# chrischoy/DeepGlobalRegistration

Hardware: AMD Instinct MI355X
Metric: pair registrations/sec (FCGF x2 + 1-NN + 6-D inlier net + gate + weighted Procrustes + SE(3) refinement) (higher is better)
Workload: dtype f32 results via 2 x f16 split operands (3 f16 MFMA products per MAC, f32 accumulate); k = 1 convs, kNN re-evaluation and registration in exact f32, SVD in f64

## Files before the change

deepglobalregistration_amd/csrc/kmap.hip:

```cpp
#include <string.h>

#include <algorithm>

#include "dgr_internal.h"
#include "hash.h"

constexpr int KM_THREADS = 256;

template <int D>
__device__ __forceinline__ void offset_of(int k, int ks, int ts, int32_t *delta) {
  const int half = ks >> 1;
#pragma unroll
  for (int d = 0; d < D; ++d) {
    delta[d] = ((k % ks) - half) * ts;
    k /= ks;
  }
}

template <int D>
__device__ __forceinline__ int probe(const int32_t *__restrict__ out_coords, int64_t o,
                                     const int32_t *delta, const int32_t *__restrict__ in_coords,
                                     const int32_t *__restrict__ in_table, uint32_t in_mask) {
  constexpr int NC = D + 1;
  int32_t q[NC];
  q[0] = out_coords[o * NC];
#pragma unroll
  for (int d = 0; d < D; ++d) q[1 + d] = out_coords[o * NC + 1 + d] + delta[d];
  return dgr_lookup<NC>(in_table, in_mask, in_coords, q);
}

template <int D>
__global__ void __launch_bounds__(KM_THREADS)
    kmap_search(const int32_t *__restrict__ out_coords, const int32_t *n_out_dev,
                const int32_t *__restrict__ in_coords, const int32_t *__restrict__ in_table,
                uint32_t in_mask, int ks, int ts_in, int RB, int64_t n_cap, int32_t *__restrict__ hits,
                int32_t *__restrict__ block_counts, int KW, uint32_t *mask_out, uint32_t *mask_in) {
  __shared__ int wave_cnt[KM_THREADS / 64];
  const int rb = blockIdx.x, k = blockIdx.y;
  const int n_out = *n_out_dev;
  if (rb * KM_THREADS >= n_out) {
    if (threadIdx.x == 0) block_counts[(int64_t)k * RB + rb] = 0;
    return;
  }
  int32_t delta[D];
  offset_of<D>(k, ks, ts_in, delta);
  const int64_t o = (int64_t)rb * KM_THREADS + threadIdx.x;
  int hit = -1;
  if (o < n_out) {
    hit = probe<D>(out_coords, o, delta, in_coords, in_table, in_mask);
    hits[(int64_t)k * n_cap + o] = hit;
    if (hit >= 0) {
      atomicOr(&mask_out[o * KW + (k >> 5)], 1u << (k & 31));
      if (mask_in) atomicOr(&mask_in[(int64_t)hit * KW + (k >> 5)], 1u << (k & 31));
    }
  }
  unsigned long long m = __ballot(hit >= 0);
  if ((threadIdx.x & 63) == 0) wave_cnt[threadIdx.x >> 6] = __popcll(m);
  __syncthreads();
  if (threadIdx.x == 0) {
    int s = 0;
#pragma unroll
    for (int w = 0; w < KM_THREADS / 64; ++w) s += wave_cnt[w];
    block_counts[(int64_t)k * RB + rb] = s;
  }
}

__device__ __forceinline__ int mask_rank(const uint32_t *__restrict__ m, int k) {
  int r = 0;
  const int w = k >> 5;
  for (int i = 0; i < w; ++i) r += __popc(m[i]);
  return r + __popc(m[w] & ((1u << (k & 31)) - 1u));
}

__global__ void mask_count_kernel(const uint32_t *__restrict__ mask, int KW, const int32_t *n_dev, int64_t n_cap,
                                  int32_t *__restrict__ cnt, unsigned short *__restrict__ wpre = nullptr) {
  const int64_t r = (int64_t)blockIdx.x * blockDim.x + threadIdx.x;
  if (r >= n_cap) return;
  int c = 0;
  if (r < *n_dev)
    for (int i = 0; i < KW; ++i) {
      if (wpre) wpre[r * KW + i] = (unsigned short)c;
      c += __popc(mask[r * KW + i]);
    }
  cnt[r] = c;
}
constexpr int KM_MC_JOBS = 8;
struct MaskCountJobs {
  const uint32_t *mask[KM_MC_JOBS];
  const int32_t *n_dev[KM_MC_JOBS];
  long long n_cap[KM_MC_JOBS];
  int32_t *cnt[KM_MC_JOBS];
  unsigned short *wpre[KM_MC_JOBS];
};
template <int KW>
__global__ void mask_count_multi(MaskCountJobs J) {
  const int m = blockIdx.y;
  const int64_t r = (int64_t)blockIdx.x * blockDim.x + threadIdx.x;
  if (r >= J.n_cap[m]) return;
  int c = 0;
  if (r < *J.n_dev[m]) {
    uint32_t w[KW];
#pragma unroll
    for (int i = 0; i < KW; ++i) w[i] = J.mask[m][r * KW + i];
#pragma unroll
    for (int i = 0; i < KW; ++i) {
      J.wpre[m][r * KW + i] = (unsigned short)c;
      c += __popc(w[i]);
    }
  }
  J.cnt[m][r] = c;
}
__device__ __forceinline__ int mask_rank_pre(const uint32_t *__restrict__ m, const unsigned short *__restrict__ pre, int k) {
  return pre[k >> 5] + __popc(m[k >> 5] & ((1u << (k & 31)) - 1u));
}


__device__ __forceinline__ unsigned long long hit_pack(int k, int64_t o, int64_t in) {
  return ((unsigned long long)k << 54) | ((unsigned long long)o << 27) | (unsigned long long)in;
}
constexpr int KM_REGION = 512;
constexpr int KM_JOBS6 = 8;
struct HitList {
  unsigned long long *recs;
  int32_t *wave_count;
  int region;
};
__device__ __forceinline__ void hit_begin(volatile int *cur) {
  if ((threadIdx.x & 63) == 0) cur[threadIdx.x >> 6] = 0;
}
__device__ __forceinline__ int64_t hit_slots(int n, const HitList &h, volatile int *cur, int wave_id) {
  const unsigned long long act = __ballot(1), two = __ballot(n == 2);
  const int lane = threadIdx.x & 63, w = threadIdx.x >> 6;
  const unsigned long long below = (1ull << lane) - 1ull;
  int base = 0;
  if (lane == __ffsll((long long)act) - 1) {
    base = cur[w];
    const int need = __popcll(act) + __popcll(two);
    if (base >= 0 && base + need <= h.region) {
      cur[w] = base + need;
    } else {
      cur[w] = -1;
      base = -1;
    }
  }
  base = __builtin_amdgcn_readfirstlane(base);
  if (base < 0) return -1;
  return (int64_t)wave_id * h.region + base + __popcll(act & below) + __popcll(two & below);
}
__device__ __forceinline__ void hit_end(const HitList &h, volatile int *cur, int wave_id) {
  if ((threadIdx.x & 63) == 0) h.wave_count[wave_id] = cur[threadIdx.x >> 6];
}

struct PrunedArgs {
  const int32_t *out_coords, *n_out_dev;
  const int4 *out_order;
  int64_t n_cap;
  DgrHalfBuckets hb;
  int ts_in, symmetric;
};
template <class Emit>
__device__ __forceinline__ void pruned_search6(const PrunedArgs &a, int64_t t, Emit &&emit) {
  const int NJ = a.symmetric ? 14 : 27;
  const int ts_in = a.ts_in;
  const int ja = (int)(t / a.n_cap);
  const int64_t p = t - (int64_t)ja * a.n_cap;
  int b = -1;
  int64_t o = 0;
  int c4 = 0, c5 = 0, c6 = 0;
  if (ja < NJ && p < *a.n_out_dev) {
    const int4 me = a.out_order[p];
    o = me.w; c4 = me.x; c5 = me.y; c6 = me.z;
    const int32_t *co = a.out_coords + o * 7;
    int32_t q[4];
    q[0] = co[0];
    q[1] = co[1] + ((ja % 3) - 1) * ts_in;
    q[2] = co[2] + (((ja / 3) % 3) - 1) * ts_in;
    q[3] = co[3] + ((ja / 9) - 1) * ts_in;
    b = dgr_lookup<4>(a.hb.table, a.hb.mask, a.hb.bkeys, q);
  }
  const int beg = b >= 0 ? a.hb.start[b] : 0, end = b >= 0 ? a.hb.start[b + 1] : 0;
  for (int p0 = beg; p0 < end; p0 += 4) {
    int4 e[4];
#pragma unroll
    for (int u = 0; u < 4; ++u) e[u] = a.hb.second[min(p0 + u, end - 1)];
#pragma unroll
    for (int u = 0; u < 4; ++u) {
      if (p0 + u >= end) break;
      const int d4 = e[u].x - c4, d5 = e[u].y - c5, d6 = e[u].z - c6;
      if (abs(d4) <= ts_in && abs(d5) <= ts_in && abs(d6) <= ts_in) {
        const int k = ja + 27 * ((d4 / ts_in + 1) + 3 * (d5 / ts_in + 1) + 9 * (d6 / ts_in + 1));
        if (a.symmetric && ja == 13 && k > 364) continue;
        emit(k, o, e[u].w);
      }
    }
  }
}

struct Bits6Jobs {
  PrunedArgs pa[KM_JOBS6];
  uint32_t *mask_out[KM_JOBS6], *mask_in[KM_JOBS6];
  HitList hl[KM_JOBS6];
  int blocks[KM_JOBS6];
};
__global__ void __launch_bounds__(KM_THREADS)
    kmap_bits_pruned6(Bits6Jobs J, int KW) {
  __shared__ int hit_cur[KM_THREADS / 64];
  const int jm = blockIdx.y;
  if ((int)blockIdx.x >= J.blocks[jm]) return;
  const PrunedArgs a = J.pa[jm];
  uint32_t *const mask_out = J.mask_out[jm], *const mask_in = J.mask_in[jm];
  const HitList hl = J.hl[jm];
  hit_begin(hit_cur);
  const int wid = (int)(blockIdx.x * (KM_THREADS / 64) + (threadIdx.x >> 6));
  pruned_search6(a, (int64_t)blockIdx.x * KM_THREADS + threadIdx.x, [&](int k, int64_t o, int in) {
    atomicOr(&mask_out[o * KW + (k >> 5)], 1u << (k & 31));
    const int km = 728 - k;
    if (a.symmetric) {
      if (km != k) atomicOr(&mask_out[(int64_t)in * KW + (km >> 5)], 1u << (km & 31));
    } else if (mask_in) {
      atomicOr(&mask_in[(int64_t)in * KW + (k >> 5)], 1u << (k & 31));
    }
    const int n = (a.symmetric && km != k) ? 2 : 1;
    const int64_t s = hit_slots(n, hl, hit_cur, wid);
    if (s >= 0) {
      hl.recs[s] = hit_pack(k, o, in);
      if (n == 2) hl.recs[s + 1] = hit_pack(km, in, o);
    }
  });
  hit_end(hl, hit_cur, wid);
}

constexpr int KM_KMAX = 736;
struct Colmask6Jobs {
  const uint32_t *mask_out[KM_JOBS6];
  const int32_t *n_out_dev[KM_JOBS6];
  int RB[KM_JOBS6];
  int4 *cell[KM_JOBS6];
  int32_t *counts[KM_JOBS6], *row_cnt[KM_JOBS6];
  unsigned short *wpre[KM_JOBS6];
};
__global__ void __launch_bounds__(KM_THREADS)
    kmap_colmask(Colmask6Jobs J, int K, int KW) {
  __shared__ unsigned long long bal[KM_THREADS / 64][KM_KMAX];
  const int jm = blockIdx.y;
  const int RB = J.RB[jm];
  if ((int)blockIdx.x >= RB) return;
  const uint32_t *__restrict__ mask_out = J.mask_out[jm];
  const int32_t *n_out_dev = J.n_out_dev[jm];
  int4 *__restrict__ cell = J.cell[jm];
  int32_t *__restrict__ counts = J.counts[jm], *__restrict__ row_cnt = J.row_cnt[jm];
  unsigned short *__restrict__ wpre = J.wpre[jm];
  const int rb = blockIdx.x;
  const int lane = threadIdx.x & 63, wave = threadIdx.x >> 6;
  const int n_out = *n_out_dev;
  const int64_t o = (int64_t)rb * KM_THREADS + threadIdx.x;
  int row_pairs = 0;
  constexpr int KW_MAX = (KM_KMAX + 31) / 32;
  uint32_t words[KW_MAX];
#pragma unroll
  for (int w = 0; w < KW_MAX; ++w) words[w] = (w < KW && o < n_out) ? mask_out[o * KW + w] : 0u;
#pragma unroll
  for (int w = 0; w < KW_MAX; ++w) {
    if (w < KW) {
      const uint32_t word = words[w];
      if (o < n_out) wpre[o * KW + w] = (unsigned short)row_pairs;
      row_pairs += __popc(word);
      unsigned long long mine = 0;
#pragma unroll
      for (int b = 0; b < 32; ++b) {
        const unsigned long long m = __ballot((word >> b) & 1u);
        if (lane == b) mine = m;
      }
      if (lane < 32 && 32 * w + lane < KM_KMAX) bal[wave][32 * w + lane] = mine;
    }
  }
  if (o < n_out) row_cnt[o] = row_pairs;
  __syncthreads();
  for (int k = threadIdx.x; k < K; k += KM_THREADS) {
    int run = 0;
#pragma unroll
    for (int g = 0; g < KM_THREADS / 64; ++g) {
      const unsigned long long m = bal[g][k];
      cell[((int64_t)rb * (KM_THREADS / 64) + g) * K + k] = make_int4((int)(m & 0xffffffffull), (int)(m >> 32), run, 0);
      run += __popcll(m);
    }
    counts[(int64_t)k * RB + rb] = run;
  }
}

struct PlaceArgs {
  int K, KW, RB;
  const uint32_t *mask_out;
  const int32_t *out_ptr;
  const int4 *cell;
  const int32_t *base;
  int32_t *pair_in, *pair_out;
  uint16_t *pair_k;
  int32_t *out_pos;
  int64_t pair_cap;
  int32_t *overflow;
  const uint32_t *mask_in;
  const int32_t *in_ptr;
  int32_t *in_pos;
  const unsigned short *wpre_out, *wpre_in;
};
__device__ __forceinline__ void place_pair(const PlaceArgs &p, int k, int64_t o, int64_t in) {
  const int64_t slot = (int64_t)p.out_ptr[o] + mask_rank_pre(p.mask_out + o * p.KW, p.wpre_out + o * p.KW, k);
  const int64_t g = o >> 6;
  const int4 c = p.cell[g * p.K + k];
  const unsigned long long cm = ((unsigned long long)(uint32_t)c.y << 32) | (uint32_t)c.x;
  const int64_t pos = (int64_t)p.base[(int64_t)k * p.RB + (g >> 2)] + c.z + __popcll(cm & ((1ull << (o & 63)) - 1ull));
  if (pos < p.pair_cap && slot < p.pair_cap) {
    p.pair_in[pos] = (int32_t)in;
    if (p.pair_out) p.pair_out[pos] = (int32_t)o;
    if (p.pair_k) p.pair_k[pos] = (uint16_t)k;
    p.out_pos[slot] = (int32_t)pos;
    if (p.mask_in) p.in_pos[p.in_ptr[in] + mask_rank_pre(p.mask_in + in * p.KW, p.wpre_in + in * p.KW, k)] = (int32_t)pos;
  } else {
    *p.overflow = 2;
  }
}

struct Place6Jobs {
  HitList h[KM_JOBS6];
  PlaceArgs p[KM_JOBS6];
  PrunedArgs replay[KM_JOBS6];
  int n_waves[KM_JOBS6], blocks[KM_JOBS6];
};
__global__ void __launch_bounds__(KM_THREADS)
    kmap_place_hits(Place6Jobs J) {
  const int jm = blockIdx.y;
  const int nblk = J.blocks[jm];
  if ((int)blockIdx.x >= nblk) return;
  const HitList h = J.h[jm];
  const PlaceArgs p = J.p[jm];
  const PrunedArgs replay = J.replay[jm];
  const int n_waves = J.n_waves[jm];
  const int lane = threadIdx.x & 63;
  for (int r = blockIdx.x * (KM_THREADS / 64) + (threadIdx.x >> 6); r < n_waves; r += nblk * (KM_THREADS / 64)) {
    const int n = h.wave_count[r];
    if (n < 0) {
      pruned_search6(replay, (int64_t)r * 64 + lane, [&](int k, int64_t o, int in) {
        place_pair(p, k, o, in);
        if (replay.symmetric && 728 - k != k) place_pair(p, 728 - k, in, o);
      });
      continue;
    }
    for (int e = lane; e < n; e += 64) {
      const unsigned long long rec = h.recs[(int64_t)r * h.region + e];
      place_pair(p, (int)(rec >> 54), (int64_t)((rec >> 27) & 0x7ffffffull), (int64_t)(rec & 0x7ffffffull));
    }
  }
}

constexpr int KM_KGROUP = 8;
__global__ void __launch_bounds__(KM_THREADS)
    kmap_fill(const int32_t *n_out_dev, int RB, int K, int64_t n_cap, const int32_t *__restrict__ hits,
              const int32_t *__restrict__ block_counts, const int32_t *__restrict__ block_base,
              int32_t *__restrict__ pair_in, int32_t *__restrict__ pair_out, int64_t pair_cap,
              int32_t *overflow, int KW, const uint32_t *__restrict__ mask_out,
              const int32_t *__restrict__ out_ptr, int32_t *__restrict__ out_pos,
              const uint32_t *__restrict__ mask_in, const int32_t *__restrict__ in_ptr,
              int32_t *__restrict__ in_pos, uint16_t *__restrict__ pair_k) {
  __shared__ int wave_cnt[2][KM_THREADS / 64];
  const int rb = blockIdx.x;
  const int n_out = *n_out_dev;
  if (rb * KM_THREADS >= n_out) return;
  const int lane = threadIdx.x & 63, wave = threadIdx.x >> 6;
  const int64_t o = (int64_t)rb * KM_THREADS + threadIdx.x;
  int parity = 0;
  for (int kk = 0; kk < KM_KGROUP; ++kk) {
    const int k = blockIdx.y * KM_KGROUP + kk;
    if (k >= K) break;
    const int64_t cell = (int64_t)k * RB + rb;
    if (block_counts[cell] == 0) continue;
    int hit = -1;
    if (o < n_out) hit = hits[(int64_t)k * n_cap + o];
    const unsigned long long m = __ballot(hit >= 0);
    if (lane == 0) wave_cnt[parity][wave] = __popcll(m);
    __syncthreads();
    if (hit >= 0) {
      int base = block_base[cell];
      for (int w = 0; w < wave; ++w) base += wave_cnt[parity][w];
      const int64_t pos = base + __popcll(m & ((1ull << lane) - 1ull));
      if (pos < pair_cap) {
        pair_in[pos] = hit;
        if (pair_out) pair_out[pos] = (int32_t)o;
        if (pair_k) pair_k[pos] = (uint16_t)k;
        out_pos[out_ptr[o] + mask_rank(mask_out + o * KW, k)] = (int32_t)pos;
        if (mask_in) in_pos[in_ptr[hit] + mask_rank(mask_in + (int64_t)hit * KW, k)] = (int32_t)pos;
      } else {
        *overflow = 2;
      }
    }
    parity ^= 1;
  }
}

constexpr int KM_MAXJOBS = 8;
struct FinalizeJobs {
  const int32_t *base[KM_MAXJOBS], *total[KM_MAXJOBS];
  int32_t *rule_ptr[KM_MAXJOBS], *tile_ptr[KM_MAXJOBS];
  int4 *desc[KM_MAXJOBS];
  long long tile_cap[KM_MAXJOBS];
  int K[KM_MAXJOBS], RB[KM_MAXJOBS];
};
__global__ void __launch_bounds__(1024) kmap_finalize(FinalizeJobs j) {
  __shared__ int s[1024];
  const int m = blockIdx.x, K = j.K[m], RB = j.RB[m];
  const int32_t *block_base = j.base[m];
  const int k = threadIdx.x;
  int start = 0, end = 0;
  if (k < K) {
    start = block_base[(int64_t)k * RB];
    end = (k + 1 < K) ? block_base[(int64_t)(k + 1) * RB] : *j.total[m];
    j.rule_ptr[m][k] = start;
    if (k == K - 1) j.rule_ptr[m][K] = end;
  }
  const int tiles = (end - start + DGR_TILE_M - 1) / DGR_TILE_M;
  s[k] = tiles;
  __syncthreads();
  for (int d = 1; d < 1024; d <<= 1) {
    const int v = (k >= d) ? s[k - d] : 0;
    __syncthreads();
    s[k] += v;
    __syncthreads();
  }
  if (k < K) j.tile_ptr[m][k] = s[k] - tiles;
  if (k == K - 1) j.tile_ptr[m][K] = s[k];
}

__device__ __forceinline__ void tile_desc_one(const int32_t *__restrict__ tile_ptr, const int32_t *__restrict__ rule_ptr, int K,
                                              int4 *__restrict__ desc, int64_t tile_cap, int64_t t, int tile_m) {
  if (t >= tile_cap || t >= tile_ptr[K]) return;
  int lo = 0, hi = K;
  while (hi - lo > 1) {
    const int mid = (lo + hi) >> 1;
    if (tile_ptr[mid] <= t) lo = mid; else hi = mid;
  }
  const int pstart = rule_ptr[lo] + ((int)t - tile_ptr[lo]) * tile_m;
  desc[t] = make_int4(lo, pstart, min(tile_m, rule_ptr[lo + 1] - pstart), 0);
}
__global__ void tile_desc_kernel(FinalizeJobs j) {
  const int m = blockIdx.y;
  const int64_t t = (int64_t)blockIdx.x * blockDim.x + threadIdx.x;
  tile_desc_one(j.tile_ptr[m], j.rule_ptr[m], j.K[m], j.desc[m], j.tile_cap[m], t, DGR_TILE_M);
}

static int alloc_kernel_map(DgrArena &arena, int K, int64_t n_cap, int64_t n_in_cap, int max_pairs_per_row, bool need_in_csr,
                            bool want_pair_out, bool want_pair_k, DgrKernelMap *km) {
  DGR_REQUIRE(K <= 1024, "kernel volume %d > 1024 not supported", K);
  km->K = K;
  const int64_t per_row = K < max_pairs_per_row ? K : max_pairs_per_row;
  km->pair_cap = per_row * n_cap;
  DGR_REQUIRE(km->pair_cap < (1ll << 31), "kernel map too large (%lld pairs)", (long long)km->pair_cap);
  DGR_ALLOC(km->rule_ptr, arena, int32_t, K + 1);
  DGR_ALLOC(km->tile_ptr, arena, int32_t, K + 1);
  DGR_ALLOC(km->pair_in, arena, int32_t, km->pair_cap);
  km->pair_out = nullptr;
  if (want_pair_out) DGR_ALLOC(km->pair_out, arena, int32_t, km->pair_cap);
  km->tile_cap = km->pair_cap / DGR_TILE_M + K;
  DGR_ALLOC(km->tile_desc, arena, int4, km->tile_cap);
  DGR_ALLOC(km->out_ptr, arena, int32_t, n_cap + 1);
  DGR_ALLOC(km->out_pos, arena, int32_t, km->pair_cap);
  km->pair_k = nullptr;
  if (want_pair_k) DGR_ALLOC(km->pair_k, arena, uint16_t, km->pair_cap);
  if (need_in_csr) {
    DGR_ALLOC(km->in_ptr, arena, int32_t, n_in_cap + 1);
    DGR_ALLOC(km->in_pos, arena, int32_t, km->pair_cap);
  }
  return DGR_OK;
}

static void finalize_job(FinalizeJobs &fj, int m, const int32_t *base, const int32_t *total, int K, int RB, DgrKernelMap *km) {
  fj.base[m] = base; fj.total[m] = total; fj.K[m] = K; fj.RB[m] = RB;
  fj.rule_ptr[m] = km->rule_ptr; fj.tile_ptr[m] = km->tile_ptr;
  fj.desc[m] = km->tile_desc; fj.tile_cap[m] = km->tile_cap;
}

static int build_kernel_map3(DgrArena &arena, const DgrCoordMap &in, const DgrCoordMap &out, int ks, int max_pairs_per_row,
                             bool need_in_csr, bool want_pair_out, bool want_pair_k, DgrKernelMap *km,
                             int32_t *overflow, hipStream_t stream) {
  constexpr int D = 3;
  const int K = ks * ks * ks;
  const int64_t n_cap = out.n_cap, n_in_cap = in.n_cap;
  const int RB = (int)dgr_ceil_div(n_cap, KM_THREADS);
  DGR_CHECK(alloc_kernel_map(arena, K, n_cap, n_in_cap, max_pairs_per_row, need_in_csr, want_pair_out, want_pair_k, km));
  const int KW = (K + 31) / 32;
  DgrArena::Mark mk = arena.mark();
  int32_t *counts, *base, *total;
  DGR_ALLOC(counts, arena, int32_t, (int64_t)K * RB);
  DGR_ALLOC(base, arena, int32_t, (int64_t)K * RB);
  DGR_ALLOC(total, arena, int32_t, 1);
  uint32_t *mask_out, *mask_in = nullptr;
  int32_t *cnt_out, *cnt_in = nullptr;
  {
    const size_t w_out = (size_t)(n_cap + 1) * KW, w_in = need_in_csr ? (size_t)(n_in_cap + 1) * KW : 0;
    DGR_ALLOC(mask_out, arena, uint32_t, w_out + w_in);
    if (need_in_csr) mask_in = mask_out + w_out;
    DGR_HIP_CHECK(hipMemsetAsync(mask_out, 0, (w_out + w_in) * sizeof(uint32_t), stream));
  }
  DGR_ALLOC(cnt_out, arena, int32_t, n_cap + 1);
  if (need_in_csr) DGR_ALLOC(cnt_in, arena, int32_t, n_in_cap + 1);
  int32_t *hits;
  DGR_ALLOC(hits, arena, int32_t, (int64_t)K * n_cap);
  kmap_search<D><<<dim3(RB, K), KM_THREADS, 0, stream>>>(out.coords, out.n_dev, in.coords, in.table, in.table_mask, ks,
                                                         in.ts, RB, n_cap, hits, counts, KW, mask_out, mask_in);
  DGR_LAUNCH_CHECK();
  mask_count_kernel<<<(int)dgr_ceil_div(n_cap + 1, 256), 256, 0, stream>>>(mask_out, KW, out.n_dev, n_cap + 1, cnt_out);
  if (need_in_csr)
    mask_count_kernel<<<(int)dgr_ceil_div(n_in_cap + 1, 256), 256, 0, stream>>>(mask_in, KW, in.n_dev, n_in_cap + 1, cnt_in);
  {
    const int32_t *ins[3] = {cnt_out, counts, cnt_in};
    int32_t *outs[3] = {km->out_ptr, base, km->in_ptr}, *tots[3] = {nullptr, total, nullptr};
    const int64_t ns[3] = {n_cap + 1, (int64_t)K * RB, n_in_cap + 1};
    DGR_CHECK(dgr_exclusive_scan_multi(arena, need_in_csr ? 3 : 2, ins, outs, ns, tots, stream));
  }
  FinalizeJobs fj = {};
  finalize_job(fj, 0, base, total, K, RB, km);
  kmap_finalize<<<1, 1024, 0, stream>>>(fj);
  tile_desc_kernel<<<dim3((unsigned)dgr_ceil_div(km->tile_cap, 256), 1), 256, 0, stream>>>(fj);
  kmap_fill<<<dim3(RB, (K + KM_KGROUP - 1) / KM_KGROUP), KM_THREADS, 0, stream>>>(
      out.n_dev, RB, K, n_cap, hits, counts, base, km->pair_in, km->pair_out, km->pair_cap, overflow, KW, mask_out,
      km->out_ptr, km->out_pos, mask_in, km->in_ptr, km->in_pos, km->pair_k);
  DGR_LAUNCH_CHECK();
  arena.rewind(mk);
  km->built = true;
  return DGR_OK;
}

struct Kmap6Job {
  const DgrCoordMap *in, *out;
  const DgrHalfBuckets *hb;
  const DgrHalfBuckets *hb_out;
  bool need_in_csr, want_pair_out, want_pair_k;
  DgrKernelMap *km;
};
static int build_kernel_maps6(DgrArena &arena, const Kmap6Job *jobs, int nj, int max_pairs_per_row, int32_t *overflow,
                              hipStream_t stream) {
  constexpr int K = 729, KW = (K + 31) / 32;
  DGR_REQUIRE(nj >= 1 && nj <= KM_MAXJOBS, "6-D kernel maps: %d jobs", nj);
  struct Tr {
    int RB, symmetric;
    int64_t n_cap, n_in_cap, hit_waves;
    int32_t *counts, *base, *total, *cnt_out, *cnt_in;
    uint32_t *mask_out, *mask_in;
    int4 *cell;
    HitList hl;
    unsigned short *wpre_out, *wpre_in;
  } t[KM_MAXJOBS];
  for (int m = 0; m < nj; ++m) {
    const Kmap6Job &J = jobs[m];
    t[m].n_cap = J.out->n_cap; t[m].n_in_cap = J.in->n_cap;
    DGR_REQUIRE(t[m].n_cap < (1ll << 27) && t[m].n_in_cap < (1ll << 27), "6-D kernel maps: more than 2^27 rows");
    DGR_CHECK(alloc_kernel_map(arena, K, t[m].n_cap, t[m].n_in_cap, max_pairs_per_row, J.need_in_csr, J.want_pair_out,
                               J.want_pair_k, J.km));
  }
  DgrArena::Mark mk = arena.mark();
  {
    size_t words = 0;
    for (int m = 0; m < nj; ++m)
      words += (size_t)(t[m].n_cap + 1) * KW + (jobs[m].need_in_csr ? (size_t)(t[m].n_in_cap + 1) * KW : 0) + (size_t)(t[m].n_cap + 1);
    uint32_t *pool;
    DGR_ALLOC(pool, arena, uint32_t, words);
    DGR_HIP_CHECK(hipMemsetAsync(pool, 0, words * sizeof(uint32_t), stream));
    for (int m = 0; m < nj; ++m) {
      t[m].mask_out = pool; pool += (size_t)(t[m].n_cap + 1) * KW;
      t[m].mask_in = nullptr;
      if (jobs[m].need_in_csr) { t[m].mask_in = pool; pool += (size_t)(t[m].n_in_cap + 1) * KW; }
      t[m].cnt_out = reinterpret_cast<int32_t *>(pool); pool += (size_t)(t[m].n_cap + 1);
    }
  }
  for (int m = 0; m < nj; ++m) {
    const Kmap6Job &J = jobs[m];
    Tr &r = t[m];
    r.RB = (int)dgr_ceil_div(r.n_cap, KM_THREADS);
    r.symmetric = (J.in->coords == J.out->coords && !J.need_in_csr) ? 1 : 0;
    DGR_REQUIRE(J.hb && J.hb->built && J.hb_out && J.hb_out->built, "6-D kernel map: first-half buckets missing");
    DGR_ALLOC(r.counts, arena, int32_t, (int64_t)K * r.RB);
    DGR_ALLOC(r.base, arena, int32_t, (int64_t)K * r.RB);
    DGR_ALLOC(r.total, arena, int32_t, 1);
    r.cnt_in = nullptr;
    if (J.need_in_csr) DGR_ALLOC(r.cnt_in, arena, int32_t, r.n_in_cap + 1);
    DGR_ALLOC(r.cell, arena, int4, (int64_t)r.RB * (KM_THREADS / 64) * K);
    const int64_t search_blocks = dgr_ceil_div(r.n_cap * (r.symmetric ? 14 : 27), KM_THREADS);
    r.hit_waves = search_blocks * (KM_THREADS / 64);
    r.hl.region = (J.in->ts >= 8 && r.symmetric) ? 2 * KM_REGION : KM_REGION / 2;
    DGR_REQUIRE(r.hit_waves < (1ll << 31), "6-D kernel map: too many search waves");
    DGR_ALLOC(r.hl.recs, arena, unsigned long long, r.hit_waves * r.hl.region);
    DGR_ALLOC(r.hl.wave_count, arena, int32_t, r.hit_waves);
    DGR_ALLOC(r.wpre_out, arena, unsigned short, (r.n_cap + 1) * KW);
    r.wpre_in = nullptr;
    if (J.need_in_csr) DGR_ALLOC(r.wpre_in, arena, unsigned short, (r.n_in_cap + 1) * KW);
  }
  static_assert(KM_JOBS6 >= KM_MAXJOBS, "multi-job launch tables");
  {
    Bits6Jobs bj = {};
    Colmask6Jobs cj = {};
    int max_sb = 0, max_rb = 0;
    for (int m = 0; m < nj; ++m) {
      const Kmap6Job &J = jobs[m];
      Tr &r = t[m];
      bj.pa[m] = PrunedArgs{J.out->coords, J.out->n_dev, J.hb_out->second, r.n_cap, *J.hb, J.in->ts, r.symmetric};
      bj.mask_out[m] = r.mask_out; bj.mask_in[m] = r.mask_in; bj.hl[m] = r.hl;
      bj.blocks[m] = (int)(r.hit_waves / (KM_THREADS / 64));
      max_sb = std::max(max_sb, bj.blocks[m]);
      cj.mask_out[m] = r.mask_out; cj.n_out_dev[m] = J.out->n_dev; cj.RB[m] = r.RB; cj.cell[m] = r.cell;
      cj.counts[m] = r.counts; cj.row_cnt[m] = r.cnt_out; cj.wpre[m] = r.wpre_out;
      max_rb = std::max(max_rb, r.RB);
    }
    kmap_bits_pruned6<<<dim3((unsigned)max_sb, (unsigned)nj), KM_THREADS, 0, stream>>>(bj, KW);
    kmap_colmask<<<dim3((unsigned)max_rb, (unsigned)nj), KM_THREADS, 0, stream>>>(cj, K, KW);
    {
      MaskCountJobs mj = {};
      int nm = 0;
      long long max_rows = 0;
      for (int m = 0; m < nj; ++m)
        if (jobs[m].need_in_csr) {
          mj.mask[nm] = t[m].mask_in; mj.n_dev[nm] = jobs[m].in->n_dev; mj.n_cap[nm] = t[m].n_in_cap + 1;
          mj.cnt[nm] = t[m].cnt_in; mj.wpre[nm] = t[m].wpre_in;
          max_rows = std::max(max_rows, mj.n_cap[nm]);
          ++nm;
        }
      static_assert(KM_MC_JOBS >= KM_MAXJOBS, "mask-count job table");
      if (nm) mask_count_multi<KW><<<dim3((unsigned)dgr_ceil_div(max_rows, 256), (unsigned)nm), 256, 0, stream>>>(mj);
    }
  }
  DGR_LAUNCH_CHECK();
  {
    const int32_t *ins[DGR_SCAN_MAX];
    int32_t *outs[DGR_SCAN_MAX], *tots[DGR_SCAN_MAX];
    int64_t ns[DGR_SCAN_MAX];
    int c = 0;
    for (int m = 0; m < nj; ++m) {
      ins[c] = t[m].cnt_out; outs[c] = jobs[m].km->out_ptr; tots[c] = nullptr; ns[c++] = t[m].n_cap + 1;
      ins[c] = t[m].counts; outs[c] = t[m].base; tots[c] = t[m].total; ns[c++] = (int64_t)K * t[m].RB;
      if (jobs[m].need_in_csr) { ins[c] = t[m].cnt_in; outs[c] = jobs[m].km->in_ptr; tots[c] = nullptr; ns[c++] = t[m].n_in_cap + 1; }
    }
    DGR_CHECK(dgr_exclusive_scan_multi(arena, c, ins, outs, ns, tots, stream));
  }
  FinalizeJobs fj = {};
  int64_t max_tiles = 0;
  for (int m = 0; m < nj; ++m) {
    finalize_job(fj, m, t[m].base, t[m].total, K, t[m].RB, jobs[m].km);
    max_tiles = std::max<int64_t>(max_tiles, jobs[m].km->tile_cap);
  }
  kmap_finalize<<<nj, 1024, 0, stream>>>(fj);
  tile_desc_kernel<<<dim3((unsigned)dgr_ceil_div(max_tiles, 256), nj), 256, 0, stream>>>(fj);
  {
    Place6Jobs pj = {};
    int max_pb = 0;
    for (int m = 0; m < nj; ++m) {
      const Kmap6Job &J = jobs[m];
      Tr &r = t[m];
      DgrKernelMap *km = J.km;
      pj.p[m] = PlaceArgs{K, KW, r.RB, r.mask_out, km->out_ptr, r.cell, r.base, km->pair_in, km->pair_out, km->pair_k, km->out_pos,
                          km->pair_cap, overflow, r.mask_in, km->in_ptr, km->in_pos, r.wpre_out, r.wpre_in};
      pj.replay[m] = PrunedArgs{J.out->coords, J.out->n_dev, J.hb_out->second, r.n_cap, *J.hb, J.in->ts, r.symmetric};
      pj.h[m] = r.hl;
      pj.n_waves[m] = (int)r.hit_waves;
      pj.blocks[m] = (int)std::min<int64_t>(dgr_ceil_div(r.hit_waves, KM_THREADS / 64), 16384);
      max_pb = std::max(max_pb, pj.blocks[m]);
      km->built = true;
    }
    kmap_place_hits<<<dim3((unsigned)max_pb, (unsigned)nj), KM_THREADS, 0, stream>>>(pj);
  }
  DGR_LAUNCH_CHECK();
  arena.rewind(mk);
  return DGR_OK;
}

constexpr int NBR_JOBS = 10;
struct NbrJobs {
  const int32_t *out_coords[NBR_JOBS], *n_out_dev[NBR_JOBS], *in_coords[NBR_JOBS], *in_table[NBR_JOBS];
  uint32_t in_mask[NBR_JOBS];
  int ts[NBR_JOBS];
  long long n_pad[NBR_JOBS];
  int32_t *nbr[NBR_JOBS];
};
__global__ void __launch_bounds__(KM_THREADS) nbr_search3(NbrJobs J) {
  const int jm = blockIdx.z;
  const int64_t n_pad = J.n_pad[jm];
  const int64_t o = (int64_t)blockIdx.x * KM_THREADS + threadIdx.x;
  if (o >= n_pad) return;
  int32_t *__restrict__ nbr = J.nbr[jm];
  const int kz = blockIdx.y;
  if (o >= *J.n_out_dev[jm]) {
#pragma unroll
    for (int u = 0; u < 9; ++u) nbr[(int64_t)(9 * kz + u) * n_pad + o] = -1;
    return;
  }
  const int sts = J.ts[jm];
  const int4 c = *reinterpret_cast<const int4 *>(J.out_coords[jm] + o * 4);
  int32_t q[9][4];
#pragma unroll
  for (int u = 0; u < 9; ++u) {
    q[u][0] = c.x;
    q[u][1] = c.y + ((u % 3) - 1) * sts;
    q[u][2] = c.z + ((u / 3) - 1) * sts;
    q[u][3] = c.w + (kz - 1) * sts;
  }
  int hit[9];
  dgr_lookup_many<4, 9>(J.in_table[jm], J.in_mask[jm], J.in_coords[jm], q, hit);
#pragma unroll
  for (int u = 0; u < 9; ++u) nbr[(int64_t)(9 * kz + u) * n_pad + o] = hit[u];
}

struct ClsJobs {
  const int32_t *coords[3], *n_dev[3];
  int ts[3], nb[3];
  int32_t *blk_cnt[3], *perm[3], *cls_count[3];
  long long cls_cap[3];
};
__device__ __forceinline__ int parity_class(const int32_t *coords, int64_t o, int ts) {
  const int4 c = *reinterpret_cast<const int4 *>(coords + o * 4);
  return ((c.y / ts) & 1) | (((c.z / ts) & 1) << 1) | (((c.w / ts) & 1) << 2);
}
__global__ void __launch_bounds__(KM_THREADS) cls_count_kernel(ClsJobs J) {
  __shared__ int wcnt[KM_THREADS / 64][8];
  const int l = blockIdx.y, b = blockIdx.x;
  if (b >= J.nb[l]) return;
  const int64_t o = (int64_t)b * KM_THREADS + threadIdx.x;
  const int cls = o < *J.n_dev[l] ? parity_class(J.coords[l], o, J.ts[l]) : 8;
#pragma unroll
  for (int c = 0; c < 8; ++c) {
    const unsigned long long m = __ballot(cls == c);
    if ((threadIdx.x & 63) == 0) wcnt[threadIdx.x >> 6][c] = __popcll(m);
  }
  __syncthreads();
  if (threadIdx.x < 8) {
    int n = 0;
    for (int w = 0; w < KM_THREADS / 64; ++w) n += wcnt[w][threadIdx.x];
    J.blk_cnt[l][b * 8 + threadIdx.x] = n;
  }
}
__global__ void __launch_bounds__(KM_THREADS) cls_fill_kernel(ClsJobs J) {
  __shared__ int part[KM_THREADS / 64][8], before[8], wcnt[KM_THREADS / 64][8];
  const int l = blockIdx.y, b = blockIdx.x;
  if (b >= J.nb[l]) return;
  const int lane = threadIdx.x & 63, wave = threadIdx.x >> 6;
  int acc[8] = {0, 0, 0, 0, 0, 0, 0, 0};
  for (int bb = threadIdx.x; bb < b; bb += KM_THREADS) {
    const int4 lo = *reinterpret_cast<const int4 *>(J.blk_cnt[l] + bb * 8), hi = *reinterpret_cast<const int4 *>(J.blk_cnt[l] + bb * 8 + 4);
    acc[0] += lo.x; acc[1] += lo.y; acc[2] += lo.z; acc[3] += lo.w;
    acc[4] += hi.x; acc[5] += hi.y; acc[6] += hi.z; acc[7] += hi.w;
  }
#pragma unroll
  for (int c = 0; c < 8; ++c) {
    int v = acc[c];
    for (int d = 32; d > 0; d >>= 1) v += __shfl_down(v, d, 64);
    if (lane == 0) part[wave][c] = v;
  }
  const int64_t o = (int64_t)b * KM_THREADS + threadIdx.x;
  const int cls = o < *J.n_dev[l] ? parity_class(J.coords[l], o, J.ts[l]) : 8;
  int rank = 0;
#pragma unroll
  for (int c = 0; c < 8; ++c) {
    const unsigned long long m = __ballot(cls == c);
    if (lane == 0) wcnt[wave][c] = __popcll(m);
    if (cls == c) rank = __popcll(m & ((1ull << lane) - 1ull));
  }
  __syncthreads();
  if (threadIdx.x < 8) {
    int n = 0;
    for (int w = 0; w < KM_THREADS / 64; ++w) n += part[w][threadIdx.x];
    before[threadIdx.x] = n;
    if (b == J.nb[l] - 1) {
      for (int w = 0; w < KM_THREADS / 64; ++w) n += wcnt[w][threadIdx.x];
      J.cls_count[l][threadIdx.x] = n;
    }
  }
  __syncthreads();
  if (cls < 8) {
    int pos = before[cls] + rank;
    for (int w = 0; w < wave; ++w) pos += wcnt[w][cls];
    J.perm[l][(int64_t)cls * J.cls_cap[l] + pos] = (int32_t)o;
  }
}

static int build_nbr_table(DgrArena &arena, const DgrCoordMap &in, const DgrCoordMap &out, int ts, int sign,
                           DgrNbrTable *t, NbrJobs *jobs, int *nj, int32_t *cls_count = nullptr) {
  t->K = 27;
  t->n_pad = dgr_ceil_div(out.n_cap, DGR_OS_ROWS) * DGR_OS_ROWS;
  DGR_ALLOC(t->nbr, arena, int32_t, t->n_pad * 27);
  t->perm = nullptr; t->cls_count = nullptr; t->cls_cap = 0;
  if (cls_count) {
    t->cls_cap = t->n_pad;
    t->cls_count = cls_count;
    DGR_ALLOC(t->perm, arena, int32_t, 8 * t->cls_cap);
  }
  DGR_REQUIRE(*nj < NBR_JOBS, "neighbour tables: more than %d per launch", NBR_JOBS);
  const int m = (*nj)++;
  jobs->out_coords[m] = out.coords; jobs->n_out_dev[m] = out.n_dev; jobs->in_coords[m] = in.coords;
  jobs->in_table[m] = in.table; jobs->in_mask[m] = in.table_mask; jobs->ts[m] = sign > 0 ? ts : -ts;
  jobs->n_pad[m] = t->n_pad; jobs->nbr[m] = t->nbr;
  t->built = true;
  return DGR_OK;
}
static int nbr_tables_launch(const NbrJobs &jobs, int nj, hipStream_t stream) {
  long long n_max = 0;
  for (int m = 0; m < nj; ++m) n_max = std::max(n_max, jobs.n_pad[m]);
  if (nj == 0) return DGR_OK;
  nbr_search3<<<dim3((unsigned)dgr_ceil_div(n_max, KM_THREADS), 3, (unsigned)nj), KM_THREADS, 0, stream>>>(jobs);
  DGR_LAUNCH_CHECK();
  return DGR_OK;
}

__global__ void nbr_count_kernel(const int32_t *__restrict__ nbr, int64_t n_pad, const int32_t *n_out_dev,
                                 unsigned long long *__restrict__ counts) {
  const int k = blockIdx.y;
  const int n = *n_out_dev;
  int c = 0;
  for (int64_t o = (int64_t)blockIdx.x * blockDim.x + threadIdx.x; o < n; o += (int64_t)gridDim.x * blockDim.x)
    c += nbr[(int64_t)k * n_pad + o] >= 0;
  for (int d = 32; d > 0; d >>= 1) c += __shfl_down(c, d, 64);
  if ((threadIdx.x & 63) == 0 && c) atomicAdd(&counts[k], (unsigned long long)c);
}

// ... 242 lines not shown
```

Before: 395.3.

## Replace per-hit record lists with per-row staged neighbor search in 6-D kmap

```diff
diff --git a/deepglobalregistration_amd/csrc/kmap.hip b/deepglobalregistration_amd/csrc/kmap.hip
--- a/deepglobalregistration_amd/csrc/kmap.hip
+++ b/deepglobalregistration_amd/csrc/kmap.hip
@@ -114,130 +114,138 @@
   return pre[k >> 5] + __popc(m[k >> 5] & ((1u << (k & 31)) - 1u));
 }
 
-
-__device__ __forceinline__ unsigned long long hit_pack(int k, int64_t o, int64_t in) {
-  return ((unsigned long long)k << 54) | ((unsigned long long)o << 27) | (unsigned long long)in;
-}
-constexpr int KM_REGION = 512;
 constexpr int KM_JOBS6 = 8;
-struct HitList {
-  unsigned long long *recs;
-  int32_t *wave_count;
-  int region;
-};
-__device__ __forceinline__ void hit_begin(volatile int *cur) {
-  if ((threadIdx.x & 63) == 0) cur[threadIdx.x >> 6] = 0;
-}
-__device__ __forceinline__ int64_t hit_slots(int n, const HitList &h, volatile int *cur, int wave_id) {
-  const unsigned long long act = __ballot(1), two = __ballot(n == 2);
-  const int lane = threadIdx.x & 63, w = threadIdx.x >> 6;
-  const unsigned long long below = (1ull << lane) - 1ull;
-  int base = 0;
-  if (lane == __ffsll((long long)act) - 1) {
-    base = cur[w];
-    const int need = __popcll(act) + __popcll(two);
-    if (base >= 0 && base + need <= h.region) {
-      cur[w] = base + need;
-    } else {
-      cur[w] = -1;
-      base = -1;
-    }
-  }
-  base = __builtin_amdgcn_readfirstlane(base);
-  if (base < 0) return -1;
-  return (int64_t)wave_id * h.region + base + __popcll(act & below) + __popcll(two & below);
-}
-__device__ __forceinline__ void hit_end(const HitList &h, volatile int *cur, int wave_id) {
-  if ((threadIdx.x & 63) == 0) h.wave_count[wave_id] = cur[threadIdx.x >> 6];
-}
-
-struct PrunedArgs {
+constexpr int KM_KMAX = 736;
+constexpr int KM_WAVE_ROWS = 8;
+
+struct RowStage {
+  int32_t *in, *spill_in;
+  uint16_t *k, *spill_k;
+  unsigned long long *spill_cur;
+  int32_t *row_spill;
+  int64_t spill_cap;
+  int width;
+};
+
+struct SearchArgs {
   const int32_t *out_coords, *n_out_dev;
   const int4 *out_order;
-  int64_t n_cap;
   DgrHalfBuckets hb;
-  int ts_in, symmetric;
-};
-template <class Emit>
-__device__ __forceinline__ void pruned_search6(const PrunedArgs &a, int64_t t, Emit &&emit) {
-  const int NJ = a.symmetric ? 14 : 27;
-  const int ts_in = a.ts_in;
-  const int ja = (int)(t / a.n_cap);
-  const int64_t p = t - (int64_t)ja * a.n_cap;
-  int b = -1;
-  int64_t o = 0;
-  int c4 = 0, c5 = 0, c6 = 0;
-  if (ja < NJ && p < *a.n_out_dev) {
+  int ts_in;
+};
+struct Search6Jobs {
+  SearchArgs a[KM_JOBS6];
+  uint32_t *mask_out[KM_JOBS6], *mask_in[KM_JOBS6];
+  RowStage st[KM_JOBS6];
+  int blocks[KM_JOBS6];
+};
+__global__ void __launch_bounds__(64)
+    kmap_search_rows6(Search6Jobs J, int KW, int32_t *overflow) {
+  __shared__ int32_t hit_in[KM_KMAX];
+  __shared__ uint32_t mask[KM_KMAX / 32 + 1];
+  __shared__ int wpre[KM_KMAX / 32 + 1];
+  __shared__ int bbeg[27], bcum[27];
+  __shared__ int64_t spill_base;
+  const int jm = blockIdx.y;
+  if ((int)blockIdx.x >= J.blocks[jm]) return;
+  const SearchArgs a = J.a[jm];
+  uint32_t *const mask_out = J.mask_out[jm], *const mask_in = J.mask_in[jm];
+  const RowStage st = J.st[jm];
+  const int lane = threadIdx.x, ts_in = a.ts_in;
+  const int n_out = *a.n_out_dev;
+  for (int i = 0; i < KM_WAVE_ROWS; ++i) {
+    const int64_t p = (int64_t)blockIdx.x * KM_WAVE_ROWS + i;
+    if (p >= n_out) break;
     const int4 me = a.out_order[p];
-    o = me.w; c4 = me.x; c5 = me.y; c6 = me.z;
-    const int32_t *co = a.out_coords + o * 7;
-    int32_t q[4];
-    q[0] = co[0];
-    q[1] = co[1] + ((ja % 3) - 1) * ts_in;
-    q[2] = co[2] + (((ja / 3) % 3) - 1) * ts_in;
-    q[3] = co[3] + ((ja / 9) - 1) * ts_in;
-    b = dgr_lookup<4>(a.hb.table, a.hb.mask, a.hb.bkeys, q);
-  }
-  const int beg = b >= 0 ? a.hb.start[b] : 0, end = b >= 0 ? a.hb.start[b + 1] : 0;
-  for (int p0 = beg; p0 < end; p0 += 4) {
-    int4 e[4];
-#pragma unroll
-    for (int u = 0; u < 4; ++u) e[u] = a.hb.second[min(p0 + u, end - 1)];
-#pragma unroll
-    for (int u = 0; u < 4; ++u) {
-      if (p0 + u >= end) break;
-      const int d4 = e[u].x - c4, d5 = e[u].y - c5, d6 = e[u].z - c6;
+    const int64_t o = me.w;
+    int size = 0;
+    if (lane < 27) {
+      const int32_t *co = a.out_coords + o * 7;
+      int32_t q[4];
+      q[0] = co[0];
+      q[1] = co[1] + ((lane % 3) - 1) * ts_in;
+      q[2] = co[2] + (((lane / 3) % 3) - 1) * ts_in;
+      q[3] = co[3] + ((lane / 9) - 1) * ts_in;
+      const int b = dgr_lookup<4>(a.hb.table, a.hb.mask, a.hb.bkeys, q);
+      if (b >= 0) {
+        const int beg = a.hb.start[b];
+        size = a.hb.start[b + 1] - beg;
+        bbeg[lane] = beg;
+      }
+    }
+    int cum = size;
+#pragma unroll
+    for (int d = 1; d < 32; d <<= 1) {
+      const int v = __shfl_up(cum, d, 64);
+      if (lane >= d) cum += v;
+    }
+    if (lane < 27) bcum[lane] = cum;
+    if (lane < KM_KMAX / 32 + 1) mask[lane] = 0u;
+    __syncthreads();
+    const int total = bcum[26];
+    for (int c = lane; c < total; c += 64) {
+      int ja = 0;
+#pragma unroll
+      for (int s = 16; s > 0; s >>= 1)
+        if (ja + s <= 26 && bcum[ja + s - 1] <= c) ja += s;
+      const int4 e = a.hb.second[bbeg[ja] + c - (ja ? bcum[ja - 1] : 0)];
+      const int d4 = e.x - me.x, d5 = e.y - me.y, d6 = e.z - me.z;
       if (abs(d4) <= ts_in && abs(d5) <= ts_in && abs(d6) <= ts_in) {
         const int k = ja + 27 * ((d4 / ts_in + 1) + 3 * (d5 / ts_in + 1) + 9 * (d6 / ts_in + 1));
-        if (a.symmetric && ja == 13 && k > 364) continue;
-        emit(k, o, e[u].w);
+        atomicOr(&mask[k >> 5], 1u << (k & 31));
+        hit_in[k] = e.w;
+        if (mask_in) atomicOr(&mask_in[(int64_t)e.w * KW + (k >> 5)], 1u << (k & 31));
       }
     }
-  }
-}
-
-struct Bits6Jobs {
-  PrunedArgs pa[KM_JOBS6];
-  uint32_t *mask_out[KM_JOBS6], *mask_in[KM_JOBS6];
-  HitList hl[KM_JOBS6];
-  int blocks[KM_JOBS6];
-};
-__global__ void __launch_bounds__(KM_THREADS)
-    kmap_bits_pruned6(Bits6Jobs J, int KW) {
-  __shared__ int hit_cur[KM_THREADS / 64];
-  const int jm = blockIdx.y;
-  if ((int)blockIdx.x >= J.blocks[jm]) return;
-  const PrunedArgs a = J.pa[jm];
-  uint32_t *const mask_out = J.mask_out[jm], *const mask_in = J.mask_in[jm];
-  const HitList hl = J.hl[jm];
-  hit_begin(hit_cur);
-  const int wid = (int)(blockIdx.x * (KM_THREADS / 64) + (threadIdx.x >> 6));
-  pruned_search6(a, (int64_t)blockIdx.x * KM_THREADS + threadIdx.x, [&](int k, int64_t o, int in) {
-    atomicOr(&mask_out[o * KW + (k >> 5)], 1u << (k & 31));
-    const int km = 728 - k;
-    if (a.symmetric) {
-      if (km != k) atomicOr(&mask_out[(int64_t)in * KW + (km >> 5)], 1u << (km & 31));
-    } else if (mask_in) {
-      atomicOr(&mask_in[(int64_t)in * KW + (k >> 5)], 1u << (k & 31));
-    }
-    const int n = (a.symmetric && km != k) ? 2 : 1;
-    const int64_t s = hit_slots(n, hl, hit_cur, wid);
-    if (s >= 0) {
-      hl.recs[s] = hit_pack(k, o, in);
-      if (n == 2) hl.recs[s + 1] = hit_pack(km, in, o);
-    }
-  });
-  hit_end(hl, hit_cur, wid);
-}
-
-constexpr int KM_KMAX = 736;
+    __syncthreads();
+    const uint32_t word = lane < KW ? mask[lane] : 0u;
+    int incl = __popc(word);
+#pragma unroll
+    for (int d = 1; d < 32; d <<= 1) {
+      const int v = __shfl_up(incl, d, 64);
+      if (lane >= d) incl += v;
+    }
+    if (lane < KW) {
+      wpre[lane] = incl - __popc(word);
+      mask_out[o * KW + lane] = word;
+    }
+    const int cnt = __shfl(incl, 31, 64);
+    if (cnt > st.width && lane == 0) {
+      int64_t base = (int64_t)atomicAdd(st.spill_cur, (unsigned long long)(cnt - st.width));
+      if (base + cnt - st.width > st.spill_cap) {
+        *overflow = 2;
+        base = st.spill_cap;
+      }
+      st.row_spill[o] = (int32_t)base;
+      spill_base = base;
+    }
+    __syncthreads();
+    for (int k = lane; k < KM_KMAX; k += 64) {
+      const uint32_t w = mask[k >> 5];
+      if ((w >> (k & 31)) & 1u) {
+        const int r = wpre[k >> 5] + __popc(w & ((1u << (k & 31)) - 1u));
+        if (r < st.width) {
+          st.in[o * st.width + r] = hit_in[k];
+          st.k[o * st.width + r] = (uint16_t)k;
+        } else {
+          const int64_t s = spill_base + r - st.width;
+          if (s < st.spill_cap) {
+            st.spill_in[s] = hit_in[k];
+            st.spill_k[s] = (uint16_t)k;
+          }
+        }
+      }
+    }
+    __syncthreads();
+  }
+}
+
 struct Colmask6Jobs {
   const uint32_t *mask_out[KM_JOBS6];
   const int32_t *n_out_dev[KM_JOBS6];
   int RB[KM_JOBS6];
   int4 *cell[KM_JOBS6];
   int32_t *counts[KM_JOBS6], *row_cnt[KM_JOBS6];
-  unsigned short *wpre[KM_JOBS6];
 };
 __global__ void __launch_bounds__(KM_THREADS)
     kmap_colmask(Colmask6Jobs J, int K, int KW) {
@@ -249,7 +257,6 @@
   const int32_t *n_out_dev = J.n_out_dev[jm];
   int4 *__restrict__ cell = J.cell[jm];
   int32_t *__restrict__ counts = J.counts[jm], *__restrict__ row_cnt = J.row_cnt[jm];
-  unsigned short *__restrict__ wpre = J.wpre[jm];
   const int rb = blockIdx.x;
   const int lane = threadIdx.x & 63, wave = threadIdx.x >> 6;
   const int n_out = *n_out_dev;
@@ -263,7 +270,6 @@
   for (int w = 0; w < KW_MAX; ++w) {
     if (w < KW) {
       const uint32_t word = words[w];
-      if (o < n_out) wpre[o * KW + w] = (unsigned short)row_pairs;
       row_pairs += __popc(word);
       unsigned long long mine = 0;
 #pragma unroll
@@ -290,7 +296,7 @@
 
 struct PlaceArgs {
   int K, KW, RB;
-  const uint32_t *mask_out;
+  const int32_t *n_out_dev;
   const int32_t *out_ptr;
   const int4 *cell;
   const int32_t *base;
@@ -298,57 +304,52 @@
   uint16_t *pair_k;
   int32_t *out_pos;
   int64_t pair_cap;
-  int32_t *overflow;
   const uint32_t *mask_in;
   const int32_t *in_ptr;
   int32_t *in_pos;
-  const unsigned short *wpre_out, *wpre_in;
-};
-__device__ __forceinline__ void place_pair(const PlaceArgs &p, int k, int64_t o, int64_t in) {
-  const int64_t slot = (int64_t)p.out_ptr[o] + mask_rank_pre(p.mask_out + o * p.KW, p.wpre_out + o * p.KW, k);
+  const unsigned short *wpre_in;
+  RowStage st;
+};
+struct Place6Jobs {
+  PlaceArgs p[KM_JOBS6];
+  int blocks[KM_JOBS6];
+};
+__global__ void __launch_bounds__(KM_THREADS)
+    kmap_place_rows6(Place6Jobs J, int32_t *overflow) {
+  const int jm = blockIdx.y;
+  if ((int)blockIdx.x >= J.blocks[jm]) return;
+  const PlaceArgs p = J.p[jm];
+  const int lane = threadIdx.x & 63;
+  const int64_t o = (int64_t)blockIdx.x * (KM_THREADS / 64) + (threadIdx.x >> 6);
+  if (o >= *p.n_out_dev) return;
+  const int64_t beg = p.out_ptr[o];
+  const int cnt = (int)(p.out_ptr[o + 1] - beg);
   const int64_t g = o >> 6;
-  const int4 c = p.cell[g * p.K + k];
-  const unsigned long long cm = ((unsigned long long)(uint32_t)c.y << 32) | (uint32_t)c.x;
-  const int64_t pos = (int64_t)p.base[(int64_t)k * p.RB + (g >> 2)] + c.z + __popcll(cm & ((1ull << (o & 63)) - 1ull));
-  if (pos < p.pair_cap && slot < p.pair_cap) {
-    p.pair_in[pos] = (int32_t)in;
-    if (p.pair_out) p.pair_out[pos] = (int32_t)o;
-    if (p.pair_k) p.pair_k[pos] = (uint16_t)k;
-    p.out_pos[slot] = (int32_t)pos;
-    if (p.mask_in) p.in_pos[p.in_ptr[in] + mask_rank_pre(p.mask_in + in * p.KW, p.wpre_in + in * p.KW, k)] = (int32_t)pos;
-  } else {
-    *p.overflow = 2;
-  }
-}
-
-struct Place6Jobs {
-  HitList h[KM_JOBS6];
-  PlaceArgs p[KM_JOBS6];
-  PrunedArgs replay[KM_JOBS6];
-  int n_waves[KM_JOBS6], blocks[KM_JOBS6];
-};
-__global__ void __launch_bounds__(KM_THREADS)
-    kmap_place_hits(Place6Jobs J) {
-  const int jm = blockIdx.y;
-  const int nblk = J.blocks[jm];
-  if ((int)blockIdx.x >= nblk) return;
-  const HitList h = J.h[jm];
-  const PlaceArgs p = J.p[jm];
-  const PrunedArgs replay = J.replay[jm];
-  const int n_waves = J.n_waves[jm];
-  const int lane = threadIdx.x & 63;
-  for (int r = blockIdx.x * (KM_THREADS / 64) + (threadIdx.x >> 6); r < n_waves; r += nblk * (KM_THREADS / 64)) {
-    const int n = h.wave_count[r];
-    if (n < 0) {
-      pruned_search6(replay, (int64_t)r * 64 + lane, [&](int k, int64_t o, int in) {
-        place_pair(p, k, o, in);
-        if (replay.symmetric && 728 - k != k) place_pair(p, 728 - k, in, o);
-      });
-      continue;
-    }
-    for (int e = lane; e < n; e += 64) {
-      const unsigned long long rec = h.recs[(int64_t)r * h.region + e];
-      place_pair(p, (int)(rec >> 54), (int64_t)((rec >> 27) & 0x7ffffffull), (int64_t)(rec & 0x7ffffffull));
+  const unsigned long long below = (1ull << (o & 63)) - 1ull;
+  for (int r = lane; r < cnt; r += 64) {
+    int64_t in;
+    int k;
+    if (r < p.st.width) {
+      in = p.st.in[o * p.st.width + r];
+      k = p.st.k[o * p.st.width + r];
+    } else {
+      const int64_t s = (int64_t)p.st.row_spill[o] + r - p.st.width;
+      if (s >= p.st.spill_cap) continue;
+      in = p.st.spill_in[s];
+      k = p.st.spill_k[s];
+    }
+    const int4 c = p.cell[g * p.K + k];
+    const unsigned long long cm = ((unsigned long long)(uint32_t)c.y << 32) | (uint32_t)c.x;
+    const int64_t pos = (int64_t)p.base[(int64_t)k * p.RB + (g >> 2)] + c.z + __popcll(cm & below);
+    const int64_t slot = beg + r;
+    if (pos < p.pair_cap && slot < p.pair_cap) {
+      p.pair_in[pos] = (int32_t)in;
+      if (p.pair_out) p.pair_out[pos] = (int32_t)o;
+      if (p.pair_k) p.pair_k[pos] = (uint16_t)k;
+      p.out_pos[slot] = (int32_t)pos;
+      if (p.mask_in) p.in_pos[p.in_ptr[in] + mask_rank_pre(p.mask_in + in * p.KW, p.wpre_in + in * p.KW, k)] = (int32_t)pos;
+    } else {
+      *overflow = 2;
     }
   }
 }
@@ -541,18 +542,17 @@
   constexpr int K = 729, KW = (K + 31) / 32;
   DGR_REQUIRE(nj >= 1 && nj <= KM_MAXJOBS, "6-D kernel maps: %d jobs", nj);
   struct Tr {
-    int RB, symmetric;
-    int64_t n_cap, n_in_cap, hit_waves;
+    int RB;
+    int64_t n_cap, n_in_cap;
     int32_t *counts, *base, *total, *cnt_out, *cnt_in;
     uint32_t *mask_out, *mask_in;
     int4 *cell;
-    HitList hl;
-    unsigned short *wpre_out, *wpre_in;
+    RowStage st;
+    unsigned short *wpre_in;
   } t[KM_MAXJOBS];
   for (int m = 0; m < nj; ++m) {
     const Kmap6Job &J = jobs[m];
     t[m].n_cap = J.out->n_cap; t[m].n_in_cap = J.in->n_cap;
-    DGR_REQUIRE(t[m].n_cap < (1ll << 27) && t[m].n_in_cap < (1ll << 27), "6-D kernel maps: more than 2^27 rows");
     DGR_CHECK(alloc_kernel_map(arena, K, t[m].n_cap, t[m].n_in_cap, max_pairs_per_row, J.need_in_csr, J.want_pair_out,
                                J.want_pair_k, J.km));
   }
@@ -560,10 +560,11 @@
   {
     size_t words = 0;
     for (int m = 0; m < nj; ++m)
-      words += (size_t)(t[m].n_cap + 1) * KW + (jobs[m].need_in_csr ? (size_t)(t[m].n_in_cap + 1) * KW : 0) + (size_t)(t[m].n_cap + 1);
+      words += (size_t)(t[m].n_cap + 1) * KW + (jobs[m].need_in_csr ? (size_t)(t[m].n_in_cap + 1) * KW : 0) + (size_t)(t[m].n_cap + 1) + 2;
     uint32_t *pool;
     DGR_ALLOC(pool, arena, uint32_t, words);
     DGR_HIP_CHECK(hipMemsetAsync(pool, 0, words * sizeof(uint32_t), stream));
+    for (int m = 0; m < nj; ++m) { t[m].st.spill_cur = reinterpret_cast<unsigned long long *>(pool); pool += 2; }
     for (int m = 0; m < nj; ++m) {
       t[m].mask_out = pool; pool += (size_t)(t[m].n_cap + 1) * KW;
       t[m].mask_in = nullptr;
@@ -575,7 +576,6 @@
     const Kmap6Job &J = jobs[m];
     Tr &r = t[m];
     r.RB = (int)dgr_ceil_div(r.n_cap, KM_THREADS);
-    r.symmetric = (J.in->coords == J.out->coords && !J.need_in_csr) ? 1 : 0;
     DGR_REQUIRE(J.hb && J.hb->built && J.hb_out && J.hb_out->built, "6-D kernel map: first-half buckets missing");
     DGR_ALLOC(r.counts, arena, int32_t, (int64_t)K * r.RB);
     DGR_ALLOC(r.base, arena, int32_t, (int64_t)K * r.RB);
@@ -583,33 +583,33 @@
     r.cnt_in = nullptr;
     if (J.need_in_csr) DGR_ALLOC(r.cnt_in, arena, int32_t, r.n_in_cap + 1);
     DGR_ALLOC(r.cell, arena, int4, (int64_t)r.RB * (KM_THREADS / 64) * K);
-    const int64_t search_blocks = dgr_ceil_div(r.n_cap * (r.symmetric ? 14 : 27), KM_THREADS);
-    r.hit_waves = search_blocks * (KM_THREADS / 64);
-    r.hl.region = (J.in->ts >= 8 && r.symmetric) ? 2 * KM_REGION : KM_REGION / 2;
-    DGR_REQUIRE(r.hit_waves < (1ll << 31), "6-D kernel map: too many search waves");
-    DGR_ALLOC(r.hl.recs, arena, unsigned long long, r.hit_waves * r.hl.region);
-    DGR_ALLOC(r.hl.wave_count, arena, int32_t, r.hit_waves);
-    DGR_ALLOC(r.wpre_out, arena, unsigned short, (r.n_cap + 1) * KW);
+    r.st.width = (int)(J.km->pair_cap / r.n_cap);
+    r.st.spill_cap = J.km->pair_cap;
+    DGR_ALLOC(r.st.in, arena, int32_t, J.km->pair_cap);
+    DGR_ALLOC(r.st.k, arena, uint16_t, J.km->pair_cap);
+    DGR_ALLOC(r.st.spill_in, arena, int32_t, r.st.spill_cap);
+    DGR_ALLOC(r.st.spill_k, arena, uint16_t, r.st.spill_cap);
+    DGR_ALLOC(r.st.row_spill, arena, int32_t, r.n_cap);
     r.wpre_in = nullptr;
     if (J.need_in_csr) DGR_ALLOC(r.wpre_in, arena, unsigned short, (r.n_in_cap + 1) * KW);
   }
   static_assert(KM_JOBS6 >= KM_MAXJOBS, "multi-job launch tables");
   {
-    Bits6Jobs bj = {};
+    Search6Jobs bj = {};
     Colmask6Jobs cj = {};
     int max_sb = 0, max_rb = 0;
     for (int m = 0; m < nj; ++m) {
       const Kmap6Job &J = jobs[m];
       Tr &r = t[m];
-      bj.pa[m] = PrunedArgs{J.out->coords, J.out->n_dev, J.hb_out->second, r.n_cap, *J.hb, J.in->ts, r.symmetric};
-      bj.mask_out[m] = r.mask_out; bj.mask_in[m] = r.mask_in; bj.hl[m] = r.hl;
-      bj.blocks[m] = (int)(r.hit_waves / (KM_THREADS / 64));
+      bj.a[m] = SearchArgs{J.out->coords, J.out->n_dev, J.hb_out->second, *J.hb, J.in->ts};
+      bj.mask_out[m] = r.mask_out; bj.mask_in[m] = r.mask_in; bj.st[m] = r.st;
+      bj.blocks[m] = (int)dgr_ceil_div(r.n_cap, KM_WAVE_ROWS);
       max_sb = std::max(max_sb, bj.blocks[m]);
       cj.mask_out[m] = r.mask_out; cj.n_out_dev[m] = J.out->n_dev; cj.RB[m] = r.RB; cj.cell[m] = r.cell;
-      cj.counts[m] = r.counts; cj.row_cnt[m] = r.cnt_out; cj.wpre[m] = r.wpre_out;
+      cj.counts[m] = r.counts; cj.row_cnt[m] = r.cnt_out;
       max_rb = std::max(max_rb, r.RB);
     }
-    kmap_bits_pruned6<<<dim3((unsigned)max_sb, (unsigned)nj), KM_THREADS, 0, stream>>>(bj, KW);
+    kmap_search_rows6<<<dim3((unsigned)max_sb, (unsigned)nj), 64, 0, stream>>>(bj, KW, overflow);
     kmap_colmask<<<dim3((unsigned)max_rb, (unsigned)nj), KM_THREADS, 0, stream>>>(cj, K, KW);
     {
       MaskCountJobs mj = {};
@@ -654,16 +654,13 @@
       const Kmap6Job &J = jobs[m];
       Tr &r = t[m];
       DgrKernelMap *km = J.km;
-      pj.p[m] = PlaceArgs{K, KW, r.RB, r.mask_out, km->out_ptr, r.cell, r.base, km->pair_in, km->pair_out, km->pair_k, km->out_pos,
-                          km->pair_cap, overflow, r.mask_in, km->in_ptr, km->in_pos, r.wpre_out, r.wpre_in};
-      pj.replay[m] = PrunedArgs{J.out->coords, J.out->n_dev, J.hb_out->second, r.n_cap, *J.hb, J.in->ts, r.symmetric};
-      pj.h[m] = r.hl;
-      pj.n_waves[m] = (int)r.hit_waves;
-      pj.blocks[m] = (int)std::min<int64_t>(dgr_ceil_div(r.hit_waves, KM_THREADS / 64), 16384);
+      pj.p[m] = PlaceArgs{K, KW, r.RB, J.out->n_dev, km->out_ptr, r.cell, r.base, km->pair_in, km->pair_out, km->pair_k,
+                          km->out_pos, km->pair_cap, r.mask_in, km->in_ptr, km->in_pos, r.wpre_in, r.st};
+      pj.blocks[m] = (int)dgr_ceil_div(r.n_cap, KM_THREADS / 64);
       max_pb = std::max(max_pb, pj.blocks[m]);
       km->built = true;
     }
-    kmap_place_hits<<<dim3((unsigned)max_pb, (unsigned)nj), KM_THREADS, 0, stream>>>(pj);
+    kmap_place_rows6<<<dim3((unsigned)max_pb, (unsigned)nj), KM_THREADS, 0, stream>>>(pj, overflow);
   }
   DGR_LAUNCH_CHECK();
   arena.rewind(mk);
```

New measurement: 385.5. 2.5% lower.
